# QCLovers/PyTDSCF

Measured on AMD Instinct MI355X. Metric: tdvp_sweeps_per_sec, higher is better.
Workload: dtype c128; 1 GPU; C4: synthetic exciton chain L=64 d=16 D=1024 M=32; L=64, d=16, D=1024, M=32, integrator=lanczos, steps_per_half_sweep=8, parallelism=single, approximate=False

## Files before the change

### include/mitdvp.h

```cpp
#ifndef MITDVP_H
#define MITDVP_H

#include <stddef.h>
#include <stdint.h>

#ifdef __cplusplus
extern "C" {
#endif

typedef struct mitdvp_engine mitdvp_engine;

enum {
  MITDVP_OK = 0,
  MITDVP_EINVAL = -1,
  MITDVP_EHIP = -2,
  MITDVP_ENOTCONV = -3,
  MITDVP_ESTATE = -4,
  MITDVP_ENOMEM = -5
};

enum { MITDVP_LANCZOS = 0, MITDVP_ARNOLDI = 1 };
enum { MITDVP_GAUGE_C = -1 , MITDVP_GAUGE_PSI = 0, MITDVP_GAUGE_A = 1, MITDVP_GAUGE_B = 2 };

typedef struct {
// ... 171 lines not shown
  double env_flops, env_ms;
  double keff_flops, keff_ms;
  double qr_flops, qr_ms;
  double krylov_vec_ms;
  long long n_heff, n_keff, n_env, n_qr;
  long long n_exp_site, n_exp_bond;
  long long n_launch;
  double heff_stage_ms[3];
  double n_collectives;
  double collective_bytes;
  double heff_flops_skipped;
  double n_host_waits;
  double n_heff_edge;
  double heff_stage_flops[3];
  double n_env_fold;
} mitdvp_counters;
int mitdvp_counters_get(mitdvp_engine* h, mitdvp_counters* out);
int mitdvp_counters_reset(mitdvp_engine* h);
int mitdvp_set_profiling(mitdvp_engine* h, int on);

int mitdvp_heff_apply(int device, const double* L, const double* W, const double* R, const double* psi,
                      int dl, int d, int dr, int ml, int mr, double* sigma_out, int reps, double* ms_out);
int mitdvp_keff_apply(int device, const double* L, const double* R, const double* sval,
                      int dl, int dr, int m, double* out);
int mitdvp_env_update(int device, int left, const double* env, const double* site, const double* W,
                      int dl, int d, int dr, int ml, int mr, double* out);
int mitdvp_gauge_trf(int device, int key, const double* psi, int dl, int d, int dr,
                     double* site_out, double* sigma_out);
int mitdvp_expm_dense(int device, int integrator, int conserve_norm, int lanczos_variant,
                      const double* mat, int n, const double* x, double scale_re, double scale_im,
// ... 39 lines not shown
```

### pytdscf_amd/_lib.py

```python

from __future__ import annotations

import ctypes as C
import os
import re

_HERE = os.path.dirname(os.path.abspath(__file__))
LIB_PATH = os.environ.get("MITDVP_LIB") or os.path.join(_HERE, "csrc", "libmitdvp.so")
HEADER_PATH = os.path.join(os.path.dirname(_HERE), "include", "mitdvp.h")

OK, EINVAL, EHIP, ENOTCONV, ESTATE, ENOMEM = 0, -1, -2, -3, -4, -5
LANCZOS, ARNOLDI = 0, 1
GAUGE_PSI, GAUGE_A, GAUGE_B, GAUGE_C = 0, 1, 2, -1


class MitdvpError(RuntimeError):
    pass


class Config(C.Structure):
    _fields_ = [
        ("nsite", C.c_int),
        ("device", C.c_int),
        ("integrator", C.c_int),
# ... 23 lines not shown
        ("n_heff", C.c_longlong),
        ("n_keff", C.c_longlong),
        ("n_env", C.c_longlong),
        ("n_qr", C.c_longlong),
        ("n_exp_site", C.c_longlong),
        ("n_exp_bond", C.c_longlong),
        ("n_launch", C.c_longlong),
        ("heff_stage_ms", C.c_double * 3),
        ("n_collectives", C.c_double),
        ("collective_bytes", C.c_double),
        ("heff_flops_skipped", C.c_double),
        ("n_host_waits", C.c_double),
        ("n_heff_edge", C.c_double),
        ("heff_stage_flops", C.c_double * 3),
        ("n_env_fold", C.c_double),
    ]

    def as_dict(self):
        d = {k: getattr(self, k) for k, _ in self._fields_ if k not in ("reserved", "heff_stage_ms", "heff_stage_flops")}
        d["heff_stage_ms"] = list(self.heff_stage_ms)
        d["heff_stage_flops"] = list(self.heff_stage_flops)
        return d


class BatchOut(C.Structure):

    _fields_ = [(k, C.POINTER(C.c_double)) for k in
                ("norm", "autocorr", "energy", "rdm", "mean_norm2", "mean_autocorr", "mean_energy", "mean_rdm")]


# ... 202 lines not shown
```

### pytdscf_amd/csrc/engine.h

```cpp
#pragma once
#include <functional>
#include <map>
#include <memory>
#include <string>
#include <vector>

#include "../../include/mitdvp.h"
#include "common.h"
#include "krylov_dev.h"
#include "qr.h"
#include "small_site.h"
#include "svd.h"
#include "vecops.h"

namespace mitdvp {

struct DevBuf {
  zc* p = nullptr;
  size_t n = 0;
  DevBuf() = default;
  DevBuf(const DevBuf&) = delete;
  DevBuf& operator=(const DevBuf&) = delete;
  DevBuf(DevBuf&& o) noexcept : p(o.p), n(o.n) { o.p = nullptr; o.n = 0; }
  DevBuf& operator=(DevBuf&& o) noexcept {
// ... 33 lines not shown
};

struct MpoSite {
  int ml = 0, d = 0, mr = 0;
  DevBuf w2l;
  DevBuf w2r;
  DevBuf w2lt, w2rt, kl_l, kl_r;
  int kl_stride_l = 0, kl_stride_r = 0;
  double sp_frac_l = 1.0, sp_frac_r = 1.0;
  struct SpSeg { int r0, r1; bool dense; int tile0; };
  std::vector<SpSeg> seg_l, seg_r;
  DevBuf w2el;
  DevBuf w2er;
  std::vector<hzc> whost;
  std::vector<char> nzblk;
  struct EnvFold { std::vector<int> t0; DevBuf ws, wg; };
  struct EdgeCache {
    bool valid = false;
    unsigned long long s = 0, e = 0;
    std::vector<hzc> lam, mu;
    bool has_l = false, has_r = false;
    int skip = 0;
    DevBuf w_l, w_r;
    DevBuf w_lf, w_rf;
    bool lf_ok = false, rf_ok = false;
    EnvFold envf[2];
    void rebuild(hipStream_t st, const MpoSite& w, unsigned long long S, unsigned long long E, const std::vector<hzc>& lam,
                 const std::vector<hzc>& mu);
  };
  mutable EdgeCache edge;
  DevBuf wtr;
// ... 71 lines not shown

  std::string last_error;

  void heff_apply(const zc* L, const MpoSite& w, const zc* R, const zc* psi, zc* out, int dl, int d, int dr,
                  hzc shift, const ApplyPlan& plan = {});
  void keff_apply(const zc* L, const zc* R, const zc* sig, zc* out, int d1, int d2, int m, hzc shift,
                  const KeffCompact* kc = nullptr);
  void heff_apply_rect(const zc* L, const MpoSite& w, const zc* R, const zc* psi, zc* out, int dlo, int dli, int d,
                       int dro, int dri, const ApplyPlan& plan = {});
  void heff_apply_edge(const zc* L, const MpoSite& w, const zc* R, const zc* psi, zc* out, int dl, int d, int dr,
                       const ApplyPlan& plan);
  ApplyPlan choose_apply_forms(const zc* Lb, const MpoSite& w, const zc* Rb, int dl, int d, int dr);
  void keff_apply_rect(const zc* L, const zc* R, const zc* sig, zc* out, int dlo, int dli, int dro, int dri, int m);
  void env_update_rect(const zc* env_in, const zc* Tk, const zc* Tb, const zc* w2, zc* env_out, int dbi, int dki,
                       int min_, int d, int dbo, int dko, int mout, const MpoSite* sp = nullptr, int sp_side = 0);
  bool env_fold_ok(const zc* env_in, int din, int min_, int d, int dout, int mout, const MpoSite* sp, int sp_side);
  void env_update_fold(const zc* env_in, const zc* T, zc* env_out, int din, int min_, int d, int dout, int mout,
                       const MpoSite::EnvFold& f);
  void env_update(const zc* env_in, const zc* T, const zc* w2, zc* env_out, int din, int min_, int d, int dout,
                  int mout, const zc* w2e = nullptr, const MpoSite* sp = nullptr, int sp_side = 0);
  template <class MV>
  int krylov_exp(hzc scale, MV&& matvec, zc* x, long n, int k_prev, long nsize = -1);
  template <class MV>
  int krylov_diag(MV&& matvec, zc* x, long n);
  void gauge_qr_left(const zc* psi, int dl, int d, int dr, zc* A_out, zc* sigma_out);
  void gauge_qr_right(const zc* psi, int dl, int d, int dr, zc* B_out, zc* Bt_out, zc* sigma_out);
  void ensure_work(long max_site, long max_x, long max_y, int max_qr_m, int max_qr_n, int qr_next = 0);
  void set_gate(int isite, const double* reim, int d);
  void apply_gates();
  void set_kraus(int isite, int two_site, const double* reim, int k, int d);
  void apply_kraus();
  double operate(int op_id, int maxstep, double conv_tol, int* iters_out);
  void set_adaptive(bool on, int dmax, int dd, double p_proj);
  void thin_to_full_A(const zc* A, int l, int c, int r, int e, zc* out);
  void thin_to_full_B(const zc* B, int l, int c, int r, int e, zc* out);
// ... 37 lines not shown
  const MpoSite& mpo(int op_id, int isite);
  mitdvp_config cfg;

 private:
  int ptr_mode_ = 0;
  struct CuClaim {
    int dev = -1, first = 0, count = 0;
    ~CuClaim() { if (dev >= 0) cu_range_release(dev, first, count); }
  } cu_claim_;
  bool qr_gauge_free_ = true;
  bool trim_identity_ = true;
  int edge_mode_ = -1;
  int fold_mode_ = -1;
  int strassen_mode_ = -1;
  bool strassen_batched_ = true;
  DevBuf str_l_, str_r_, str_v_, str_m_;
  static bool try_reserve(DevBuf& b, size_t elems);
  void strassen_side(const zc* fixed, bool fixed_is_a, const zc* psi, long ldpsi, zc* out, long hm, long hn, long hk, bool accumulate,
                     int level);
  int fold_env_mode_ = -1;
  struct EnvChecked { const MpoSite* w = nullptr; const zc* blk[2] = {nullptr, nullptr}; int n[2] = {0, 0}; } env_chk_;
  EnvChecked take_env_checked() { const EnvChecked c = env_chk_; env_chk_ = EnvChecked{}; return c; }
  struct IdentRecord { double dev[128]; hzc lam[128]; };
  static_assert(sizeof(IdentRecord) == 128 * 8 + 128 * 16 && sizeof(IdentRecord) <= 4 * NPART * sizeof(zc), "layout of the identity-check record");
  const IdentRecord& identity_sets(const zc* L, int ml, int dl, unsigned long long ms, const zc* R, int mr, int dr, unsigned long long me);
  void identity_blocks(const zc* L, int dl, int ml, const zc* R, int dr, int mr, bool* left, bool* right);
  int L_;
  hipStream_t st_ = nullptr;
  std::vector<int> dl_, dd_, dr_, gauge_;
  std::vector<DevBuf> site_;
  std::vector<std::vector<int>> sub_;
  std::vector<int> subn_;
  std::map<int, Operator> ops_;
  int center_ = -1;
  bool segment_ = false;
  int bnd_dl_ = 1, bnd_ml_ = 1, bnd_dr_ = 1, bnd_mr_ = 1;
// ... 115 lines not shown
```

### pytdscf_amd/csrc/engine.hip

```cpp
#include "engine_internal.h"
#include "engine_krylov.inc"
#include "rccl_dyn.h"

namespace mitdvp {

Engine::Engine(const mitdvp_config& c) : cfg(c), L_(c.nsite) {
  if (c.nsite < 1) throw ArgError("nsite must be >= 1");
  if (c.max_krylov < 1 || c.max_krylov > MAXK - 1) throw ArgError("max_krylov must be in [1, 20]");
  if (c.integrator != MITDVP_LANCZOS && c.integrator != MITDVP_ARNOLDI) throw ArgError("bad integrator");
  if (c.relax < 0 || c.relax > 2) throw ArgError("relax must be 0, 1 or 2");
  max_diag_krylov_ = c.max_diag_krylov > 0 ? c.max_diag_krylov : 64;
  if (const char* e = std::getenv("MITDVP_SMALL_KERNELS")) small_kernels_ = std::atoi(e) != 0;
  if (const char* e = std::getenv("MITDVP_SPARSE_W")) sparse_w_ = std::atoi(e) != 0;
  if (const char* e = std::getenv("MITDVP_TRIM_IDENTITY")) trim_identity_ = std::atoi(e) != 0;
  if (const char* e = std::getenv("MITDVP_EDGE_APPLY")) edge_mode_ = std::atoi(e);
  if (const char* e = std::getenv("MITDVP_FOLD_APPLY")) fold_mode_ = std::atoi(e);
  if (const char* e = std::getenv("MITDVP_FOLD_STRASSEN")) strassen_mode_ = std::atoi(e);
  if (const char* e = std::getenv("MITDVP_STRASSEN_BATCH")) strassen_batched_ = std::atoi(e) != 0;
  if (const char* e = std::getenv("MITDVP_FOLD_ENV")) fold_env_mode_ = std::atoi(e);
  if (const char* e = std::getenv("MITDVP_QR_GAUGE_FREE")) qr_gauge_free_ = std::atoi(e) != 0;
  if (const char* e = std::getenv("MITDVP_KEFF_IDENT")) keff_ident_ = std::atoi(e) != 0;
  int ndev = 0;
  HIP_CHECK(hipGetDeviceCount(&ndev));
  if (ndev < 1) throw HipError("no HIP device visible: the MI355X engine has no CPU fallback");
  if (c.device < 0 || c.device >= ndev) throw ArgError("bad device ordinal");
  HIP_CHECK(hipSetDevice(c.device));
  HIP_CHECK(hipDeviceGetAttribute(&n_cu_, hipDeviceAttributeMultiprocessorCount, c.device));
  if (c.cu_count > 0) {
    if (c.cu_first < 0 || c.cu_first + c.cu_count > n_cu_ || c.cu_count % 8 != 0 || c.cu_first % 8 != 0)
      throw ArgError("cu_first / cu_count: a multiple of 8 compute units inside the device (8 k units = k CUs on every XCD)");
    std::vector<uint32_t> mask((size_t)(n_cu_ + 31) / 32, 0u);
    for (int u = c.cu_first; u < c.cu_first + c.cu_count; ++u) mask[(size_t)u / 32] |= 1u << (u % 32);
    cu_range_claim(c.device, c.cu_first, c.cu_count);
    cu_claim_.dev = c.device; cu_claim_.first = c.cu_first; cu_claim_.count = c.cu_count;
// ... 279 lines not shown
  s.w2er.reserve(w2er.size());
  HIP_CHECK(hipMemcpyAsync(s.w2el.p, w2el.data(), w2el.size() * sizeof(zc), hipMemcpyHostToDevice, st_));
  HIP_CHECK(hipMemcpyAsync(s.w2er.p, w2er.data(), w2er.size() * sizeof(zc), hipMemcpyHostToDevice, st_));
  HIP_CHECK(hipStreamSynchronize(st_));
  s.set = true;
}

void Engine::set_mpo_core(int op_id, int isite, const double* reim, int ml, int dout, int din, int mr) {
  if (isite < 0 || isite >= L_) throw ArgError("set_mpo_core: bad site index");
  upload_mpo_core(op(op_id).sites[isite], reim, ml, dout, din, mr);
  if (op_id == 0) invalidate_env();
}
void Engine::set_shift(int op_id, double re, double im) { op(op_id).shift = hzc(re, im); }

void Engine::invalidate_env() {
  for (int b = 1; b < L_; ++b) {
    envL_ok_[b] = 0; envR_ok_[b] = 0;
    pool_put(std::move(envL_[b]));
    pool_put(std::move(envR_[b]));
  }
}

void Engine::ensure_work(long max_site, long max_x, long max_y, int max_qr_m, int max_qr_n, int qr_next) {
  X_.reserve(max_x);
  Y_.reserve(max_y);
  V_.reserve((size_t)MAXK * max_site);
  tmp1_.reserve(max_site);
  tmp2_.reserve(max_site);
  const size_t dd = (size_t)max_qr_n * max_qr_n;
  sig_.reserve(std::max<size_t>(dd, 1));
// ... 350 lines not shown
        cnt_.n_exp_bond += 1;
      }
      envR_ok_[p + 1] = 0;
      pool_put(std::move(envR_[p + 1]));
      ZgemmDesc g = zgemm_desc(sig_.p, site_[p + 1].p, spare.p, dr, dd_[p + 1] * dr_[p + 1], dr);
      zgemm(st_, g);
      cnt_.n_launch += 1;
      std::swap(site_[p + 1], spare);
      gauge_[p + 1] = MITDVP_GAUGE_PSI;
      center_ = p + 1;
    } else {
      gauge_qr_right(site_[p].p, dl, d, dr, spare.p, tmp2_.p, sig_.p);
      std::swap(site_[p], spare);
      gauge_[p] = MITDVP_GAUGE_B;
      envR_[p] = pool_get((size_t)dl * w.ml * dl);
      env_update(envR_[p + 1].p, tmp2_.p, w.w2r.p, envR_[p].p, dr, w.mr, d, dl, w.ml, w.w2er.p, &w, 1);
      envR_ok_[p] = 1;
      const zc* Lb = envL_[p].p;
      const zc* Rb = envR_[p].p;
      const int m = w.ml;
      if (cfg.relax != 2 && !small_bond_exp(p, Lb, Rb, dl, m, dt)) {
        const KeffCompact* kc = keff_prepare(Lb, Rb, dl, dl, m);
        auto mk = [&](const zc* in, zc* out) { keff_apply(Lb, Rb, in, out, dl, dl, m, shift, kc); };
        kprev_[p] = krylov_exp(scale_bond(dt), mk, sig_.p, (long)dl * dl, kprev_[p]);
        cnt_.n_exp_bond += 1;
      }
      envL_ok_[p] = 0;
      pool_put(std::move(envL_[p]));
      ZgemmDesc g = zgemm_desc(site_[p - 1].p, sig_.p, spare.p, dl_[p - 1] * dd_[p - 1], dl, dl);
      zgemm(st_, g);
      cnt_.n_launch += 1;
// ... 29 lines not shown
```

### pytdscf_amd/csrc/engine_apply.hip

```cpp
#include "engine_internal.h"

namespace mitdvp {

constexpr long STRASSEN_MIN_TILES = 256;

double Engine::w_stage(const MpoSite* sp, int side, const zc* w2, int d, int mout, int min_, int ncol, int nbatch) {
  ZgemmDesc g = zgemm_desc(w2, X_.p, Y_.p, d * mout, ncol, min_ * d);
  g.batch = nbatch; g.strideA = 0; g.strideB = (long)min_ * d * ncol; g.strideC = (long)d * mout * ncol;
  const bool use = sp && sparse_w_ && ncol >= 64 && (side == 0 ? sp->kl_l.p : sp->kl_r.p) &&
                   (side == 0 ? sp->sp_frac_l : sp->sp_frac_r) <= 0.6;
  if (!use) {
    zgemm(st_, g);
    return 1.0;
  }
  const zc* wt = side == 0 ? sp->w2lt.p : sp->w2rt.p;
  const int* kl = reinterpret_cast<const int*>(side == 0 ? sp->kl_l.p : sp->kl_r.p);
  const int stride = side == 0 ? sp->kl_stride_l : sp->kl_stride_r;
  const auto& segs = side == 0 ? sp->seg_l : sp->seg_r;
  const int K = min_ * d;
  for (int pass = 0; pass < 2; ++pass)
    for (const auto& sgm : segs) {
      if (sgm.dense != (pass == 0)) continue;
      ZgemmDesc h = g;
      h.A = wt + (size_t)sgm.r0 * K;
// ... 62 lines not shown
}

bool Engine::try_reserve(DevBuf& b, size_t elems) {
  if (elems <= b.n) return true;
  zc* q = nullptr;
  if (hipMalloc(&q, elems * sizeof(zc)) != hipSuccess) { (void)hipGetLastError(); return false; }
  b.release();
  b.p = q; b.n = elems;
  return true;
}

void Engine::strassen_side(const zc* fixed, bool fixed_is_a, const zc* psi, long ldpsi, zc* out, long hm, long hn, long hk,
                           bool accumulate, int level) {
  const long vr = fixed_is_a ? hk : hm, vc = fixed_is_a ? hn : hk;
  const int vset = fixed_is_a ? STRASSEN_B : STRASSEN_A;
  strassen_operands(st_, psi, ldpsi, vr, vc, str_v_.p, vset);
  int np = 7;
  long pm = hm, pn = hn, pk = hk;
  const zc* V = str_v_.p;
  zc* Mp = str_m_.p;
  if (level == 2) {
    zc* v2 = str_v_.p + 7 * vr * vc;
    strassen_operands(st_, str_v_.p, vc, vr / 2, vc / 2, v2, vset, 7, vr * vc, 7 * (vr / 2) * (vc / 2));
    np = 49; pm = hm / 2; pn = hn / 2; pk = hk / 2;
    V = v2;
    Mp = str_m_.p + 7 * hm * hn;
  }
  const zc* A = fixed_is_a ? fixed : V;
  const zc* B = fixed_is_a ? V : fixed;
  ZgemmDesc g = zgemm_desc(A, B, Mp, (int)pm, (int)pn, (int)pk);
  if (!fixed_is_a) { g.transB = 1; g.ldb = pk; }
  if (strassen_batched_) {
    g.batch = np; g.strideA = pm * pk; g.strideB = pk * pn; g.strideC = pm * pn;
    zgemm(st_, g);
  } else {
    for (int k = 0; k < np; ++k) {
      ZgemmDesc h = g;
      h.A = A + k * pm * pk; h.B = B + k * pk * pn; h.C = Mp + k * pm * pn;
      zgemm(st_, h);
    }
  }
  if (level == 2) strassen_combine(st_, Mp, pm, pn, str_m_.p, hn, false, 7, 7 * pm * pn, hm * hn);
  strassen_combine(st_, str_m_.p, hm, hn, out, ldpsi, accumulate);
  cnt_.n_launch += (level == 2 ? 4 : 2) + (strassen_batched_ ? 1 : np);
}

void Engine::heff_apply_edge(const zc* L, const MpoSite& w, const zc* R, const zc* psi, zc* out, int dl, int d, int dr,
                             const ApplyPlan& plan) {
  const int ml = w.ml, mr = w.mr;
  const MpoSite::EdgeCache& c = w.edge;
  bool first = true;
  double exe = 0.0;
  if (c.has_r && plan.fold_r && plan.strassen_r) {
    timer_begin(12);
    const bool two = plan.strassen_r == 2;
    strassen_side(str_r_.p, false, psi, (long)d * dr, out, dl / 2, (long)d * dr / 2, (long)d * dr / 2, false,
                  plan.strassen_r);
    timer_end();
    first = false;
// ... 134 lines not shown
        if (!w.nzblk[blk(in, out)]) continue;
        for (int i = 0; i < d; ++i)
          for (int j = 0; j < d; ++j) ws[((size_t)i * d + j) * mo + out] += wt[in] * Wel(in, i, j, out);
      }
    }
    for (size_t k = 0; k < f.t0.size(); ++k)
      for (int in = 0; in < mi; ++in) {
        if (((I >> in) & 1ull) || !w.nzblk[blk(in, f.t0[k])]) continue;
        for (int i = 0; i < d; ++i)
          for (int j = 0; j < d; ++j) wg[((k * d + i) * mi + in) * d + j] = Wel(in, i, j, f.t0[k]);
      }
    f.ws.reserve(ws.size());
    f.wg.reserve(wg.size());
    HIP_CHECK(hipMemcpyAsync(f.ws.p, ws.data(), ws.size() * sizeof(zc), hipMemcpyHostToDevice, st));
    HIP_CHECK(hipMemcpyAsync(f.wg.p, wg.data(), wg.size() * sizeof(zc), hipMemcpyHostToDevice, st));
    HIP_CHECK(hipStreamSynchronize(st));
  }
  HIP_CHECK(hipStreamSynchronize(st));
  s = S; e = E; this->lam = lam; this->mu = mu; valid = true;
}

ApplyPlan Engine::choose_apply_forms(const zc* Lb, const MpoSite& w, const zc* Rb, int dl, int d, int dr) {
  ApplyPlan plan;
  (void)take_env_checked();
  int a0, a1;
  const bool sharded = shard_range(dl, a0, a1);
  const int ml = w.ml, mr = w.mr;
  const bool can_fold_r = fold_mode_ != 0 && !sharded && (fold_mode_ > 0 || mr > d) && (size_t)d * dr * d * dr <= Y_.n;
  const bool can_fold_l = fold_mode_ != 0 && !sharded && (fold_mode_ > 0 || ml > d) && (size_t)dl * d * dl * d <= X_.n;
  const bool edge_cand = edge_mode_ != 0 && trim_identity_ && !w.whost.empty() && !sharded && dl >= 32 && dr >= 32 &&
// ... 35 lines not shown
  if (plan.fold_r || plan.fold_l) {
    timer_begin(11);
    if (plan.fold_r) fold_env_core(st_, Rb, w.edge.w_r.p, Y_.p, dr, mr, d, (long)d * mr, mr, 1, (long)dr * d * dr, (long)d * dr, dr, 1);
    if (plan.fold_l) fold_env_core(st_, Lb, w.edge.w_l.p, X_.p, dl, ml, d, (long)ml * d, 1, d, (long)dl * d, (long)d * dl * d, 1, d);
    const size_t quarter = (size_t)dl * d * dr / 4;
    auto tiles_fill = [](long pm, long pn) { return ((pm + 63) / 64) * ((pn + 63) / 64) >= STRASSEN_MIN_TILES; };
    auto level_of = [&](long rows, long cols, long klen) {
      if (strassen_mode_ == 0 || rows % 2 || cols % 2 || klen % 2) return 0;
      const bool four = rows % 4 == 0 && cols % 4 == 0 && klen % 4 == 0;
      if (strassen_mode_ > 0) return strassen_mode_ >= 2 && four ? 2 : 1;
      if (four && tiles_fill(rows / 4, cols / 4)) return 2;
      return tiles_fill(rows / 2, cols / 2) ? 1 : 0;
    };
    auto pack = [&](const zc* op, long n, DevBuf& f, int which, int want) {
      const long h = n / 2, q = n / 4;
      const size_t two = 7 * quarter + 49 * (quarter / 4);
      if (want == 2 && try_reserve(f, 49 * (size_t)q * q) && try_reserve(str_v_, two) && try_reserve(str_m_, two)) {
        strassen_operands2(st_, op, n, q, q, f.p, which);
        cnt_.n_launch += 1;
        return 2;
      }
      if (want == 0 || !try_reserve(f, 7 * (size_t)h * h) || !try_reserve(str_v_, 7 * quarter) || !try_reserve(str_m_, 7 * quarter))
        return 0;
      strassen_operands(st_, op, n, h, h, f.p, which);
      cnt_.n_launch += 1;
      return 1;
    };
    if (plan.fold_r) plan.strassen_r = pack(Y_.p, (long)d * dr, str_r_, STRASSEN_BT, level_of(dl, (long)d * dr, (long)d * dr));
    if (plan.fold_l) plan.strassen_l = pack(X_.p, (long)dl * d, str_l_, STRASSEN_A, level_of((long)dl * d, dr, (long)dl * d));
    timer_end();
    cnt_.n_launch += (plan.fold_r ? 1 : 0) + (plan.fold_l ? 1 : 0);
    if (std::getenv("MITDVP_EDGE_TRACE"))
      fprintf(stderr, "[mitdvp] folded sides of a site: R %s, L %s\n",
              plan.strassen_r == 2 ? "49 quarter-size products" : plan.strassen_r ? "seven half-size products" : plan.fold_r ? "plain product" : "not folded",
              plan.strassen_l == 2 ? "49 quarter-size products" : plan.strassen_l ? "seven half-size products" : plan.fold_l ? "plain product" : "not folded");
  }
  return plan;
}

void Engine::heff_apply(const zc* L, const MpoSite& w, const zc* R, const zc* psi, zc* out, int dl, int d, int dr,
                        hzc shift, const ApplyPlan& plan) {
  SmallChain sc;
  if (small_ok() && chain_heff(sc, L, w, R, dl, d, dr, false)) {
    timer_begin(10);
// ... 130 lines not shown
  }
  (void)w_stage(sp, sp_side, w2, d, mout, min_, dko, nm);
  {
    ZgemmDesc g = zgemm_desc(Tb + (size_t)m0 * d * dbo, Y_.p, env_out, dbo, mout * dko, nm * d);
    g.transA = 1; g.conjA = 1; g.lda = dbo;
    zgemm(st_, g);
  }
  timer_end();
  if (sharded) collective(COLL_ALLREDUCE, env_out, (size_t)dbo * mout * dko);
  cnt_.n_launch += 3;
  cnt_.n_env += 1;
  cnt_.env_flops += 8.0 * ((double)nm * dki * min_ * d * dko + (double)nm * dko * min_ * mout * d * d +
                           (double)nm * dbo * dko * mout * d);
}

bool Engine::env_fold_ok(const zc* env_in, int din, int min_, int d, int dout, int mout, const MpoSite* sp, int sp_side) {
  const EnvChecked chk = take_env_checked();
  int a0, a1;
  if (fold_env_mode_ == 0 || !sp || adaptive_ || shard_range(din, a0, a1)) return false;
  if (chk.w != sp || chk.blk[sp_side] != env_in || chk.n[sp_side] != din || !sp->edge.valid || sp->d != d) return false;
  if (min_ != (sp_side == 0 ? sp->ml : sp->mr) || mout != (sp_side == 0 ? sp->mr : sp->ml)) return false;
  if (min_ > 64 || mout > 64 || d > 64 || din > 65535 || dout > 65535) return false;
  const MpoSite::EnvFold& f = sp->edge.envf[sp_side];
  const double nt = (double)f.t0.size();
  if ((size_t)d * dout * d * dout > Y_.n || (size_t)din * d * dout > Y_.n || (nt > 0 && (size_t)din * d * din * d > X_.n)) return false;
  if (fold_env_mode_ > 0) return true;
  const double fresh = (double)d * d * dout * dout * din + nt * ((double)d * d * din * din * dout + (double)d * din * dout * dout);
  const double chain = (double)min_ * d * din * din * dout + (double)mout * d * din * dout * dout;
  return min_ > d && 4.0 * fresh <= 3.0 * chain;
}

void Engine::env_update_fold(const zc* env_in, const zc* T, zc* env_out, int din, int min_, int d, int dout, int mout,
                             const MpoSite::EnvFold& f) {
  timer_begin(1);
  const long ldg = (long)d * dout;
  for (int i = 0; i < d; ++i) {
    ZgemmDesc g = zgemm_desc(T + (size_t)i * dout, T + (size_t)i * dout, Y_.p + (size_t)i * dout * ldg + (size_t)i * dout, dout,
                             (d - i) * dout, din);
    g.transA = 1; g.conjA = 1; g.lda = ldg; g.ldb = ldg; g.ldc = ldg;
    zgemm(st_, g);
  }
  gram_mirror_lower(st_, Y_.p, dout, d);
  gram_env_core(st_, Y_.p, f.ws.p, env_out, dout, mout, d);
  for (size_t k = 0; k < f.t0.size(); ++k) {
    fold_env_core(st_, env_in, f.wg.p + k * (size_t)d * min_ * d, X_.p, din, min_, d, (long)min_ * d, 1, d, (long)din * d,
                  (long)d * din * d, 1, d);
    ZgemmDesc g = zgemm_desc(X_.p, T, Y_.p, din * d, dout, din * d);
    zgemm(st_, g);
    ZgemmDesc h = zgemm_desc(T, Y_.p, env_out + (size_t)f.t0[k] * dout, dout, dout, din * d);
    h.transA = 1; h.conjA = 1; h.lda = dout; h.ldc = (long)mout * dout; h.beta = make_double2(1.0, 0.0);
    zgemm(st_, h);
  }
  timer_end();
  cnt_.n_launch += d + (d > 1 ? 1 : 0) + 1 + 3 * (long long)f.t0.size();
  cnt_.n_env += 1;
  cnt_.n_env_fold += 1;
  cnt_.env_flops += 8.0 * ((double)din * din * min_ * d * dout + (double)din * dout * min_ * mout * d * d +
                           (double)din * dout * dout * mout * d);
}

void Engine::env_update(const zc* env_in, const zc* T, const zc* w2, zc* env_out, int din, int min_, int d, int dout,
                        int mout, const zc* w2e, const MpoSite* sp, int sp_side) {
  SmallChain sc;
  if (w2e && small_ok() && chain_env(sc, T, w2e, din, min_, d, dout, mout)) {
    timer_begin(1);
    small_apply(st_, ss_, sc, env_in, env_out, ss_partials(sc), make_double2(0.0, 0.0), false);
    timer_end();
    cnt_.n_launch += 1;
    cnt_.n_env += 1;
    cnt_.env_flops += 8.0 * ((double)din * din * min_ * d * dout + (double)din * dout * min_ * mout * d * d +
                             (double)din * dout * dout * mout * d);
    (void)take_env_checked();
    return;
  }
  if (env_fold_ok(env_in, din, min_, d, dout, mout, sp, sp_side)) {
    env_update_fold(env_in, T, env_out, din, min_, d, dout, mout, sp->edge.envf[sp_side]);
    return;
  }
  env_update_rect(env_in, T, T, w2, env_out, din, din, min_, d, dout, dout, mout, sp, sp_side);
}

void Engine::identity_blocks(const zc* L, int dl, int ml, const zc* R, int dr, int mr, bool* left, bool* right) {
  double* dev = reinterpret_cast<double*>(red_.p + RED_MISC);
  const double* h = reinterpret_cast<const double*>(h_red_.h + RED_MISC);
  if (L) ident_deviation(st_, L, (long)ml * dl, dl, dev);
  if (R) ident_deviation(st_, R + (size_t)(mr - 1) * dr, (long)mr * dr, dr, dev + 1);
  if (L || R) read_partials(RED_MISC, 1);
  *left = L && h[0] < 1e-13;
  *right = R && h[1] < 1e-13;
}

// ... 2 lines not shown
```

### pytdscf_amd/csrc/engine_segment.hip

```cpp
#include "engine_internal.h"
#include "engine_krylov.inc"

namespace mitdvp {

void Engine::replace_site(int i, const double* reim, int gauge) {
  if (i < 0 || i >= L_ || !site_[i].p) throw ArgError("replace_site: bad or unset site");
  const size_t e = (size_t)dl_[i] * dd_[i] * dr_[i];
  copy_in(site_[i].p, reim, e);
  gauge_[i] = gauge;
  if (gauge == MITDVP_GAUGE_PSI) center_ = i;
  else if (center_ == i) center_ = -1;
}

void Engine::reshape_site(int i, const double* reim, int l, int n, int r, int gauge) {
  if (i < 0 || i >= L_ || !site_[i].p) throw ArgError("reshape_site: bad or unset site");
  if (l < 1 || r < 1 || n != dd_[i]) throw ArgError("reshape_site: bad shape");
  if (i != 0 && i != L_ - 1) throw ArgError("reshape_site: only a block's first or last site faces a junction");
  if ((i > 0 && l != dl_[i]) || (i < L_ - 1 && r != dr_[i])) throw ArgError("reshape_site: only the outer bond may change");
  const size_t e = (size_t)l * n * r;
  site_[i].reserve(e);
  copy_in(site_[i].p, reim, e);
  dl_[i] = l; dr_[i] = r; gauge_[i] = gauge;
  if (gauge == MITDVP_GAUGE_PSI) center_ = i;
  else if (center_ == i) center_ = -1;
// ... 92 lines not shown
    cnt_.n_launch += nl; cnt_.n_qr += 1;
    std::swap(site_[p], spare);
    gauge_[p] = MITDVP_GAUGE_A;
    pool_put(std::move(envL_[p + 1]));
    envL_[p + 1] = pool_get((size_t)dr * w.mr * dr);
    env_update(envL_[p].p, site_[p].p, w.w2l.p, envL_[p + 1].p, dl, w.ml, d, dr, w.mr, w.w2el.p, &w, 0);
    envL_ok_[p + 1] = 1;
    bond_ = p + 1; bond_dim_ = dr;
  } else {
    if (!envR_ok_[p + 1]) throw ArgError("split_center: right environment missing");
    gauge_qr_right(site_[p].p, dl, d, dr, spare.p, tmp2_.p, sig_.p);
    std::swap(site_[p], spare);
    gauge_[p] = MITDVP_GAUGE_B;
    pool_put(std::move(envR_[p]));
    envR_[p] = pool_get((size_t)dl * w.ml * dl);
    env_update(envR_[p + 1].p, tmp2_.p, w.w2r.p, envR_[p].p, dr, w.mr, d, dl, w.ml, w.w2er.p, &w, 1);
    envR_ok_[p] = 1;
    bond_ = p; bond_dim_ = dl;
  }
  pool_put(std::move(spare));
  center_ = -1;
  bond_site_ = p;
}

void Engine::bond_exp(double dt) {
  require_ready();
  if (bond_ < 0) throw ArgError("bond_exp: no pending bond matrix (call split_center first)");
  const int b = bond_;
  if (!envL_ok_[b] || !envR_ok_[b]) throw ArgError("bond_exp: the environment blocks around the bond are not built");
  int d = 0, m = 0;
  env_shape(0, b, &d, &m);
// ... 155 lines not shown
```

### pytdscf_amd/csrc/vecops.h

```cpp
#pragma once
#include "common.h"

namespace mitdvp {

constexpr int NPART = 256;
constexpr int MAXK = 21;

constexpr int SMALL_VEC_EPT = 16;
constexpr long SMALL_VEC_N = 1024L * SMALL_VEC_EPT;

struct Coefs {
  zc c[MAXK];
};

int vec_blocks(long n);
void vec_dot(hipStream_t st, const zc* x, const zc* y, long n, bool conj_x, zc* out_p );
void vec_sumsq(hipStream_t st, const zc* x, long n, double* out_p );
void vec_lanczos_update(hipStream_t st, zc* v, const zc* vm1, const zc* vm2 , long n,
                        const zc* alpha_p, const double* betaprev_p, double* out_p);
void vec_lanczos_update_deferred(hipStream_t st, zc* v, const zc* ul, const zc* ulm1 , long n, const zc* alpha_raw_p,
                                 const double* nrm_all, int l, bool orthodox, double eps, double* out_p);
void vec_lanczos_step_small(hipStream_t st, zc* w, const zc* x, const zc* vl, const zc* vm2 , long n,
                            zc* alpha_p, const double* betaprev_p, double* nrm_p, double eps);
void vec_scale_inv_norm(hipStream_t st, zc* v, long n, const double* nrm_p, double eps);
// ... 7 lines not shown
void set_identity(hipStream_t st, zc* out, int rows, int cols, long ld);
void vec_copy_raw(hipStream_t st, zc* dst, const zc* src, size_t n);
void ident_deviation(hipStream_t st, const zc* blk, long ld, int n, double* out_dev);
void ident_deviation_multi(hipStream_t st, const zc* base, int nblk, long blk_stride, long ld, int n, double* out_dev,
                           zc* lam_dev, unsigned long long mask = ~0ull, bool clear = true);
void fold_env_core(hipStream_t st, const zc* env, const zc* w, zc* G, int n, int m, int d, long wi, long wj, long wm, long gi,
                   long gp, long gj, long gq);
void gram_env_core(hipStream_t st, const zc* G, const zc* ws, zc* out, int n, int m, int d);
void gram_mirror_lower(hipStream_t st, zc* G, int n, int d);
enum { STRASSEN_A = 0, STRASSEN_B = 1, STRASSEN_BT = 2 };
void strassen_operands(hipStream_t st, const zc* src, long ld, long hr, long hc, zc* dst, int which, int batch = 1,
                       long sstride = 0, long dstride = 0);
void strassen_operands2(hipStream_t st, const zc* src, long ld, long qr, long qc, zc* dst, int which);
void strassen_combine(hipStream_t st, const zc* M, long hr, long hc, zc* out, long ldo, bool accumulate, int batch = 1,
                      long mstride = 0, long ostride = 0);
void copy2d(hipStream_t st, zc* dst, long ldd, const zc* src, long lds, long rows, int cols, int zero_to, zc a,
            bool accumulate);
struct BlockList { int n; int idx[64]; zc f[64]; };
void gather_blocks(hipStream_t st, zc* dst, int n_dst, const zc* src, int m_src, long rows, int cols, const BlockList& bl);
void fill_scaled_blocks(hipStream_t st, zc* X, long ldx, int pos0, const zc* sig, long rows, int cols, const BlockList& bl);
void accum_scaled_blocks(hipStream_t st, zc* out, const zc* X, long ldx, const zc* sig, long rows, int cols, const BlockList& bl,
                         zc both);
void col_sumsq(hipStream_t st, const zc* x, long rows, int cols, double* out );
void row_sumsq(hipStream_t st, const zc* x, int rows, long cols, double* out );
void shell_sumsq(hipStream_t st, const zc* x, int n, double* out );
void transpose_batched(hipStream_t st, const zc* in, zc* out, int rows, int cols, long ldi, long ldo, int batch,
                       long in_bs, long out_bs);
void phys_diag(hipStream_t st, const zc* C, zc* out, int dl, int n, int dr, bool trace);
void permute_0213(hipStream_t st, const zc* in, zc* out, long n0, int n1, int n2, int n3);
void clock_probe(hipStream_t st, long iters, double* host_out3 );
// ... 7 lines not shown
```

### pytdscf_amd/csrc/vecops.hip

```cpp
#include "vecops.h"
#include "krylov_dev.h"

#include <algorithm>

namespace mitdvp {

__device__ __forceinline__ double wave_sum(double v) {
#pragma unroll
  for (int o = 32; o > 0; o >>= 1) v += __shfl_down(v, o, 64);
  return v;
}

__device__ __forceinline__ double block_sum(double v, double* sh ) {
  v = wave_sum(v);
  const int lane = threadIdx.x & 63, w = threadIdx.x >> 6;
  __syncthreads();
  if (lane == 0) sh[w] = v;
  __syncthreads();
  if (threadIdx.x == 0) sh[4] = sh[0] + sh[1] + sh[2] + sh[3];
  __syncthreads();
  return sh[4];
}

__device__ __forceinline__ zc sum_partials_z(const zc* p, int np, double* sh) {
// ... 1004 lines not shown
#pragma unroll
    for (int k = 0; k < 7; ++k) m[k] = M[k * blk + r * hc + c];
    zc o[4];
    o[0] = make_double2(((m[0].x + m[3].x) - m[4].x) + m[6].x, ((m[0].y + m[3].y) - m[4].y) + m[6].y);
    o[1] = make_double2(m[2].x + m[4].x, m[2].y + m[4].y);
    o[2] = make_double2(m[1].x + m[3].x, m[1].y + m[3].y);
    o[3] = make_double2(((m[0].x - m[1].x) + m[2].x) + m[5].x, ((m[0].y - m[1].y) + m[2].y) + m[5].y);
#pragma unroll
    for (int u = 0; u < 4; ++u) {
      zc* p = out + ((u >> 1) * hr + r) * ldo + (u & 1) * hc + c;
      if (acc) { const zc v = *p; o[u].x += v.x; o[u].y += v.y; }
      *p = o[u];
    }
  }
}
void strassen_operands(hipStream_t st, const zc* src, long ld, long hr, long hc, zc* dst, int which, int batch, long sstride,
                       long dstride) {
  if (hr < 1 || hc < 1 || batch < 1) return;
  if (ld < 2 * hc) throw ArgError("strassen_operands: leading dimension below the matrix width");
  if (which < 0 || which > 2) throw ArgError("strassen_operands: bad factor set");
  if (batch > 65535) throw ArgError("strassen_operands: batch above 65535");
  const dim3 grid((unsigned)((hc + 255) / 256), (unsigned)std::min<long>(hr, 32768), (unsigned)batch);
  if (which == STRASSEN_A)
    hipLaunchKernelGGL(k_strassen_operands<STRASSEN_A>, grid, dim3(256), 0, st, src, ld, hr, hc, dst, sstride, dstride);
  else if (which == STRASSEN_B)
    hipLaunchKernelGGL(k_strassen_operands<STRASSEN_B>, grid, dim3(256), 0, st, src, ld, hr, hc, dst, sstride, dstride);
  else hipLaunchKernelGGL(k_strassen_operands<STRASSEN_BT>, grid, dim3(256), 0, st, src, ld, hr, hc, dst, sstride, dstride);
  HIP_CHECK(hipGetLastError());
}
void strassen_operands2(hipStream_t st, const zc* src, long ld, long qr, long qc, zc* dst, int which) {
// ... 3 lines not shown
  const dim3 grid((unsigned)((qc + 255) / 256), (unsigned)std::min<long>(qr, 32768));
  if (which == STRASSEN_A) hipLaunchKernelGGL(k_strassen_operands2<STRASSEN_A>, grid, dim3(256), 0, st, src, ld, qr, qc, dst);
  else if (which == STRASSEN_B) hipLaunchKernelGGL(k_strassen_operands2<STRASSEN_B>, grid, dim3(256), 0, st, src, ld, qr, qc, dst);
  else hipLaunchKernelGGL(k_strassen_operands2<STRASSEN_BT>, grid, dim3(256), 0, st, src, ld, qr, qc, dst);
  HIP_CHECK(hipGetLastError());
}
void strassen_combine(hipStream_t st, const zc* M, long hr, long hc, zc* out, long ldo, bool accumulate, int batch, long mstride,
                      long ostride) {
  if (hr < 1 || hc < 1 || batch < 1) return;
  if (ldo < 2 * hc) throw ArgError("strassen_combine: leading dimension below the matrix width");
  if (batch > 65535) throw ArgError("strassen_combine: batch above 65535");
  const dim3 grid((unsigned)((hc + 255) / 256), (unsigned)std::min<long>(hr, 32768), (unsigned)batch);
  hipLaunchKernelGGL(k_strassen_combine, grid, dim3(256), 0, st, M, hr, hc, out, ldo, accumulate ? 1 : 0, mstride, ostride);
  HIP_CHECK(hipGetLastError());
}

void gram_env_core(hipStream_t st, const zc* G, const zc* ws, zc* out, int n, int m, int d) {
  if (n < 1 || d < 1) return;
  if (m < 1 || m > 64 || n > 65535 || d > 64) throw ArgError("gram_env_core: MPO bond in [1, 64], d <= 64 and bond dimension <= 65535");
  const dim3 grid((n + 63) / 64, n), block(256);
  const size_t lds = (size_t)d * 64 * sizeof(zc);
  if (m <= 16) hipLaunchKernelGGL(k_gram_env_core<4>, grid, block, lds, st, G, ws, out, n, m, d);
  else if (m <= 32) hipLaunchKernelGGL(k_gram_env_core<8>, grid, block, lds, st, G, ws, out, n, m, d);
  else hipLaunchKernelGGL(k_gram_env_core<16>, grid, block, lds, st, G, ws, out, n, m, d);
  HIP_CHECK(hipGetLastError());
}

}
```

Baseline: 0.04424 sweeps/s.

## Fuse two-level Strassen packing/combine and reuse Strassen operands in folded env update

Two-level Strassen now packs the variable operand in one step and combines the 49 products in a single kernel when the fixed operand is A. This removes an intermediate 7-block buffer and two launches. The folded environment update gains a reuse path: when the edge fold has a single term, it reuses the Strassen-packed operator from the Heff apply. That replaces the per-term fold_env_core plus zgemm chain with one Strassen product and one scaled zgemm, using a modified weight table. This adds state carried between the apply and the env update, plus new correctness conditions on the MPO sparsity pattern.

```diff
diff --git a/include/mitdvp.h b/include/mitdvp.h
--- a/include/mitdvp.h
+++ b/include/mitdvp.h
@@ -209,6 +209,7 @@
   double n_heff_edge;
   double heff_stage_flops[3];
   double n_env_fold;
+  double n_env_reuse;
 } mitdvp_counters;
 int mitdvp_counters_get(mitdvp_engine* h, mitdvp_counters* out);
 int mitdvp_counters_reset(mitdvp_engine* h);
diff --git a/pytdscf_amd/_lib.py b/pytdscf_amd/_lib.py
--- a/pytdscf_amd/_lib.py
+++ b/pytdscf_amd/_lib.py
@@ -61,6 +61,7 @@
         ("n_heff_edge", C.c_double),
         ("heff_stage_flops", C.c_double * 3),
         ("n_env_fold", C.c_double),
+        ("n_env_reuse", C.c_double),
     ]
 
     def as_dict(self):
diff --git a/pytdscf_amd/csrc/engine.h b/pytdscf_amd/csrc/engine.h
--- a/pytdscf_amd/csrc/engine.h
+++ b/pytdscf_amd/csrc/engine.h
@@ -71,7 +71,7 @@
   DevBuf w2er;
   std::vector<hzc> whost;
   std::vector<char> nzblk;
-  struct EnvFold { std::vector<int> t0; DevBuf ws, wg; };
+  struct EnvFold { std::vector<int> t0; DevBuf ws, wg; bool reuse = false; hzc reuse_alpha; DevBuf ws_reuse; };
   struct EdgeCache {
     bool valid = false;
     unsigned long long s = 0, e = 0;
@@ -173,11 +173,12 @@
   void keff_apply_rect(const zc* L, const zc* R, const zc* sig, zc* out, int dlo, int dli, int dro, int dri, int m);
   void env_update_rect(const zc* env_in, const zc* Tk, const zc* Tb, const zc* w2, zc* env_out, int dbi, int dki,
                        int min_, int d, int dbo, int dko, int mout, const MpoSite* sp = nullptr, int sp_side = 0);
-  bool env_fold_ok(const zc* env_in, int din, int min_, int d, int dout, int mout, const MpoSite* sp, int sp_side);
+  bool env_fold_ok(const zc* env_in, int din, int min_, int d, int dout, int mout, const MpoSite* sp, int sp_side,
+                   int* reuse_level);
   void env_update_fold(const zc* env_in, const zc* T, zc* env_out, int din, int min_, int d, int dout, int mout,
-                       const MpoSite::EnvFold& f);
+                       const MpoSite::EnvFold& f, int sp_side, int reuse_level, const zc* T_plain);
   void env_update(const zc* env_in, const zc* T, const zc* w2, zc* env_out, int din, int min_, int d, int dout,
-                  int mout, const zc* w2e = nullptr, const MpoSite* sp = nullptr, int sp_side = 0);
+                  int mout, const zc* w2e = nullptr, const MpoSite* sp = nullptr, int sp_side = 0, const zc* T_plain = nullptr);
   template <class MV>
   int krylov_exp(hzc scale, MV&& matvec, zc* x, long n, int k_prev, long nsize = -1);
   template <class MV>
@@ -245,12 +246,14 @@
   int fold_mode_ = -1;
   int strassen_mode_ = -1;
   bool strassen_batched_ = true;
+  bool strassen_fuse_ = true;
   DevBuf str_l_, str_r_, str_v_, str_m_;
   static bool try_reserve(DevBuf& b, size_t elems);
   void strassen_side(const zc* fixed, bool fixed_is_a, const zc* psi, long ldpsi, zc* out, long hm, long hn, long hk, bool accumulate,
                      int level);
   int fold_env_mode_ = -1;
-  struct EnvChecked { const MpoSite* w = nullptr; const zc* blk[2] = {nullptr, nullptr}; int n[2] = {0, 0}; } env_chk_;
+  bool env_reuse_ = true;
+  struct EnvChecked { const MpoSite* w = nullptr; const zc* blk[2] = {nullptr, nullptr}; int n[2] = {0, 0}; int lvl[2] = {0, 0}; } env_chk_;
   EnvChecked take_env_checked() { const EnvChecked c = env_chk_; env_chk_ = EnvChecked{}; return c; }
   struct IdentRecord { double dev[128]; hzc lam[128]; };
   static_assert(sizeof(IdentRecord) == 128 * 8 + 128 * 16 && sizeof(IdentRecord) <= 4 * NPART * sizeof(zc), "layout of the identity-check record");
diff --git a/pytdscf_amd/csrc/engine.hip b/pytdscf_amd/csrc/engine.hip
--- a/pytdscf_amd/csrc/engine.hip
+++ b/pytdscf_amd/csrc/engine.hip
@@ -17,7 +17,9 @@
   if (const char* e = std::getenv("MITDVP_FOLD_APPLY")) fold_mode_ = std::atoi(e);
   if (const char* e = std::getenv("MITDVP_FOLD_STRASSEN")) strassen_mode_ = std::atoi(e);
   if (const char* e = std::getenv("MITDVP_STRASSEN_BATCH")) strassen_batched_ = std::atoi(e) != 0;
+  if (const char* e = std::getenv("MITDVP_STRASSEN_FUSE")) strassen_fuse_ = std::atoi(e) != 0;
   if (const char* e = std::getenv("MITDVP_FOLD_ENV")) fold_env_mode_ = std::atoi(e);
+  if (const char* e = std::getenv("MITDVP_FOLD_ENV_REUSE")) env_reuse_ = std::atoi(e) != 0;
   if (const char* e = std::getenv("MITDVP_QR_GAUGE_FREE")) qr_gauge_free_ = std::atoi(e) != 0;
   if (const char* e = std::getenv("MITDVP_KEFF_IDENT")) keff_ident_ = std::atoi(e) != 0;
   int ndev = 0;
@@ -327,6 +329,7 @@
 void Engine::set_shift(int op_id, double re, double im) { op(op_id).shift = hzc(re, im); }
 
 void Engine::invalidate_env() {
+  (void)take_env_checked();
   for (int b = 1; b < L_; ++b) {
     envL_ok_[b] = 0; envR_ok_[b] = 0;
     pool_put(std::move(envL_[b]));
@@ -707,7 +710,7 @@
       std::swap(site_[p], spare);
       gauge_[p] = MITDVP_GAUGE_B;
       envR_[p] = pool_get((size_t)dl * w.ml * dl);
-      env_update(envR_[p + 1].p, tmp2_.p, w.w2r.p, envR_[p].p, dr, w.mr, d, dl, w.ml, w.w2er.p, &w, 1);
+      env_update(envR_[p + 1].p, tmp2_.p, w.w2r.p, envR_[p].p, dr, w.mr, d, dl, w.ml, w.w2er.p, &w, 1, site_[p].p);
       envR_ok_[p] = 1;
       const zc* Lb = envL_[p].p;
       const zc* Rb = envR_[p].p;
diff --git a/pytdscf_amd/csrc/engine_apply.hip b/pytdscf_amd/csrc/engine_apply.hip
--- a/pytdscf_amd/csrc/engine_apply.hip
+++ b/pytdscf_amd/csrc/engine_apply.hip
@@ -100,17 +100,23 @@
                            bool accumulate, int level) {
   const long vr = fixed_is_a ? hk : hm, vc = fixed_is_a ? hn : hk;
   const int vset = fixed_is_a ? STRASSEN_B : STRASSEN_A;
-  strassen_operands(st_, psi, ldpsi, vr, vc, str_v_.p, vset);
+  const bool fused = level == 2 && strassen_fuse_ && fixed_is_a;
   int np = 7;
   long pm = hm, pn = hn, pk = hk;
   const zc* V = str_v_.p;
   zc* Mp = str_m_.p;
-  if (level == 2) {
-    zc* v2 = str_v_.p + 7 * vr * vc;
-    strassen_operands(st_, str_v_.p, vc, vr / 2, vc / 2, v2, vset, 7, vr * vc, 7 * (vr / 2) * (vc / 2));
+  if (fused) {
+    strassen_operands2(st_, psi, ldpsi, vr / 2, vc / 2, str_v_.p, vset);
     np = 49; pm = hm / 2; pn = hn / 2; pk = hk / 2;
-    V = v2;
-    Mp = str_m_.p + 7 * hm * hn;
+  } else {
+    strassen_operands(st_, psi, ldpsi, vr, vc, str_v_.p, vset);
+    if (level == 2) {
+      zc* v2 = str_v_.p + 7 * vr * vc;
+      strassen_operands(st_, str_v_.p, vc, vr / 2, vc / 2, v2, vset, 7, vr * vc, 7 * (vr / 2) * (vc / 2));
+      np = 49; pm = hm / 2; pn = hn / 2; pk = hk / 2;
+      V = v2;
+      Mp = str_m_.p + 7 * hm * hn;
+    }
   }
   const zc* A = fixed_is_a ? fixed : V;
   const zc* B = fixed_is_a ? V : fixed;
@@ -126,9 +132,13 @@
       zgemm(st_, h);
     }
   }
-  if (level == 2) strassen_combine(st_, Mp, pm, pn, str_m_.p, hn, false, 7, 7 * pm * pn, hm * hn);
-  strassen_combine(st_, str_m_.p, hm, hn, out, ldpsi, accumulate);
-  cnt_.n_launch += (level == 2 ? 4 : 2) + (strassen_batched_ ? 1 : np);
+  if (fused) {
+    strassen_combine2(st_, Mp, pm, pn, out, ldpsi, accumulate);
+  } else {
+    if (level == 2) strassen_combine(st_, Mp, pm, pn, str_m_.p, hn, false, 7, 7 * pm * pn, hm * hn);
+    strassen_combine(st_, str_m_.p, hm, hn, out, ldpsi, accumulate);
+  }
+  cnt_.n_launch += (fused ? 2 : level == 2 ? 4 : 2) + (strassen_batched_ ? 1 : np);
 }
 
 void Engine::heff_apply_edge(const zc* L, const MpoSite& w, const zc* R, const zc* psi, zc* out, int dl, int d, int dr,
@@ -293,6 +303,26 @@
     f.wg.reserve(wg.size());
     HIP_CHECK(hipMemcpyAsync(f.ws.p, ws.data(), ws.size() * sizeof(zc), hipMemcpyHostToDevice, st));
     HIP_CHECK(hipMemcpyAsync(f.wg.p, wg.data(), wg.size() * sizeof(zc), hipMemcpyHostToDevice, st));
+    f.reuse = false;
+    std::vector<hzc> ws2;
+    if (f.t0.size() == 1) {
+      const int o = f.t0[0];
+      const hzc wo = side == 0 ? mu[o] : lam[o];
+      bool ok = (((side == 0 ? E : S) >> o) & 1ull) && wo != hzc(0.0, 0.0);
+      if (side == 1)
+        for (int c = 0; c < ml && ok; ++c) {
+          if (c == o || !((S >> c) & 1ull) || lam[c] == hzc(0.0, 0.0)) continue;
+          for (int t = 0; t < mr && ok; ++t) if (w.nzblk[(size_t)c * mr + t]) ok = false;
+        }
+      if (ok) {
+        f.reuse = true;
+        f.reuse_alpha = hzc(1.0, 0.0) / wo;
+        ws2 = ws;
+        if (side == 1) for (int ij = 0; ij < d * d; ++ij) ws2[(size_t)ij * mo + o] = hzc(0.0, 0.0);
+        f.ws_reuse.reserve(ws2.size());
+        HIP_CHECK(hipMemcpyAsync(f.ws_reuse.p, ws2.data(), ws2.size() * sizeof(zc), hipMemcpyHostToDevice, st));
+      }
+    }
     HIP_CHECK(hipStreamSynchronize(st));
   }
   HIP_CHECK(hipStreamSynchronize(st));
@@ -358,7 +388,7 @@
     };
     auto pack = [&](const zc* op, long n, DevBuf& f, int which, int want) {
       const long h = n / 2, q = n / 4;
-      const size_t two = 7 * quarter + 49 * (quarter / 4);
+      const size_t two = (strassen_fuse_ && which == STRASSEN_A ? 0 : 7 * quarter) + 49 * (quarter / 4);
       if (want == 2 && try_reserve(f, 49 * (size_t)q * q) && try_reserve(str_v_, two) && try_reserve(str_m_, two)) {
         strassen_operands2(st_, op, n, q, q, f.p, which);
         cnt_.n_launch += 1;
@@ -372,6 +402,8 @@
     };
     if (plan.fold_r) plan.strassen_r = pack(Y_.p, (long)d * dr, str_r_, STRASSEN_BT, level_of(dl, (long)d * dr, (long)d * dr));
     if (plan.fold_l) plan.strassen_l = pack(X_.p, (long)dl * d, str_l_, STRASSEN_A, level_of((long)dl * d, dr, (long)dl * d));
+    env_chk_.lvl[0] = plan.strassen_l;
+    env_chk_.lvl[1] = plan.strassen_r;
     timer_end();
     cnt_.n_launch += (plan.fold_r ? 1 : 0) + (plan.fold_l ? 1 : 0);
     if (std::getenv("MITDVP_EDGE_TRACE"))
@@ -532,8 +564,10 @@
                            (double)nm * dbo * dko * mout * d);
 }
 
-bool Engine::env_fold_ok(const zc* env_in, int din, int min_, int d, int dout, int mout, const MpoSite* sp, int sp_side) {
+bool Engine::env_fold_ok(const zc* env_in, int din, int min_, int d, int dout, int mout, const MpoSite* sp, int sp_side,
+                         int* reuse_level) {
   const EnvChecked chk = take_env_checked();
+  *reuse_level = 0;
   int a0, a1;
   if (fold_env_mode_ == 0 || !sp || adaptive_ || shard_range(din, a0, a1)) return false;
   if (chk.w != sp || chk.blk[sp_side] != env_in || chk.n[sp_side] != din || !sp->edge.valid || sp->d != d) return false;
@@ -542,6 +576,7 @@
   const MpoSite::EnvFold& f = sp->edge.envf[sp_side];
   const double nt = (double)f.t0.size();
   if ((size_t)d * dout * d * dout > Y_.n || (size_t)din * d * dout > Y_.n || (nt > 0 && (size_t)din * d * din * d > X_.n)) return false;
+  if (env_reuse_ && f.reuse) *reuse_level = chk.lvl[sp_side];
   if (fold_env_mode_ > 0) return true;
   const double fresh = (double)d * d * dout * dout * din + nt * ((double)d * d * din * din * dout + (double)d * din * dout * dout);
   const double chain = (double)min_ * d * din * din * dout + (double)mout * d * din * dout * dout;
@@ -549,7 +584,8 @@
 }
 
 void Engine::env_update_fold(const zc* env_in, const zc* T, zc* env_out, int din, int min_, int d, int dout, int mout,
-                             const MpoSite::EnvFold& f) {
+                             const MpoSite::EnvFold& f, int sp_side, int reuse_level, const zc* T_plain) {
+  const bool reuse = reuse_level >= 1;
   timer_begin(1);
   const long ldg = (long)d * dout;
   for (int i = 0; i < d; ++i) {
@@ -559,8 +595,20 @@
     zgemm(st_, g);
   }
   gram_mirror_lower(st_, Y_.p, dout, d);
-  gram_env_core(st_, Y_.p, f.ws.p, env_out, dout, mout, d);
-  for (size_t k = 0; k < f.t0.size(); ++k) {
+  gram_env_core(st_, Y_.p, reuse ? f.ws_reuse.p : f.ws.p, env_out, dout, mout, d);
+  const zc alpha = make_double2(f.reuse_alpha.real(), f.reuse_alpha.imag());
+  if (reuse && sp_side == 0) {
+    strassen_side(str_l_.p, true, T, dout, Y_.p, (long)din * d / 2, dout / 2, (long)din * d / 2, false, reuse_level);
+    ZgemmDesc h = zgemm_desc(T, Y_.p, env_out + (size_t)f.t0[0] * dout, dout, dout, din * d);
+    h.transA = 1; h.conjA = 1; h.lda = dout; h.ldc = (long)mout * dout; h.alpha = alpha; h.beta = make_double2(1.0, 0.0);
+    zgemm(st_, h);
+  } else if (reuse) {
+    strassen_side(str_r_.p, false, T_plain, (long)d * din, Y_.p, dout / 2, (long)d * din / 2, (long)d * din / 2, false, reuse_level);
+    ZgemmDesc h = zgemm_desc(T_plain, Y_.p, env_out + (size_t)f.t0[0] * dout, dout, dout, d * din);
+    h.conjA = 1; h.transB = 1; h.ldb = (long)d * din; h.ldc = (long)mout * dout; h.alpha = alpha; h.beta = make_double2(1.0, 0.0);
+    zgemm(st_, h);
+  }
+  for (size_t k = 0; !reuse && k < f.t0.size(); ++k) {
     fold_env_core(st_, env_in, f.wg.p + k * (size_t)d * min_ * d, X_.p, din, min_, d, (long)min_ * d, 1, d, (long)din * d,
                   (long)d * din * d, 1, d);
     ZgemmDesc g = zgemm_desc(X_.p, T, Y_.p, din * d, dout, din * d);
@@ -570,15 +618,16 @@
     zgemm(st_, h);
   }
   timer_end();
-  cnt_.n_launch += d + (d > 1 ? 1 : 0) + 1 + 3 * (long long)f.t0.size();
+  cnt_.n_launch += d + (d > 1 ? 1 : 0) + 1 + (reuse ? 1 : 3 * (long long)f.t0.size());
   cnt_.n_env += 1;
   cnt_.n_env_fold += 1;
+  if (reuse) cnt_.n_env_reuse += 1;
   cnt_.env_flops += 8.0 * ((double)din * din * min_ * d * dout + (double)din * dout * min_ * mout * d * d +
                            (double)din * dout * dout * mout * d);
 }
 
 void Engine::env_update(const zc* env_in, const zc* T, const zc* w2, zc* env_out, int din, int min_, int d, int dout,
-                        int mout, const zc* w2e, const MpoSite* sp, int sp_side) {
+                        int mout, const zc* w2e, const MpoSite* sp, int sp_side, const zc* T_plain) {
   SmallChain sc;
   if (w2e && small_ok() && chain_env(sc, T, w2e, din, min_, d, dout, mout)) {
     timer_begin(1);
@@ -591,8 +640,10 @@
     (void)take_env_checked();
     return;
   }
-  if (env_fold_ok(env_in, din, min_, d, dout, mout, sp, sp_side)) {
-    env_update_fold(env_in, T, env_out, din, min_, d, dout, mout, sp->edge.envf[sp_side]);
+  int reuse_level = 0;
+  if (env_fold_ok(env_in, din, min_, d, dout, mout, sp, sp_side, &reuse_level)) {
+    if (sp_side == 1 && !T_plain) reuse_level = 0;
+    env_update_fold(env_in, T, env_out, din, min_, d, dout, mout, sp->edge.envf[sp_side], sp_side, reuse_level, T_plain);
     return;
   }
   env_update_rect(env_in, T, T, w2, env_out, din, din, min_, d, dout, dout, mout, sp, sp_side);
diff --git a/pytdscf_amd/csrc/engine_segment.hip b/pytdscf_amd/csrc/engine_segment.hip
--- a/pytdscf_amd/csrc/engine_segment.hip
+++ b/pytdscf_amd/csrc/engine_segment.hip
@@ -130,7 +130,7 @@
     gauge_[p] = MITDVP_GAUGE_B;
     pool_put(std::move(envR_[p]));
     envR_[p] = pool_get((size_t)dl * w.ml * dl);
-    env_update(envR_[p + 1].p, tmp2_.p, w.w2r.p, envR_[p].p, dr, w.mr, d, dl, w.ml, w.w2er.p, &w, 1);
+    env_update(envR_[p + 1].p, tmp2_.p, w.w2r.p, envR_[p].p, dr, w.mr, d, dl, w.ml, w.w2er.p, &w, 1, site_[p].p);
     envR_ok_[p] = 1;
     bond_ = p; bond_dim_ = dl;
   }
diff --git a/pytdscf_amd/csrc/vecops.h b/pytdscf_amd/csrc/vecops.h
--- a/pytdscf_amd/csrc/vecops.h
+++ b/pytdscf_amd/csrc/vecops.h
@@ -45,6 +45,7 @@
 void strassen_operands2(hipStream_t st, const zc* src, long ld, long qr, long qc, zc* dst, int which);
 void strassen_combine(hipStream_t st, const zc* M, long hr, long hc, zc* out, long ldo, bool accumulate, int batch = 1,
                       long mstride = 0, long ostride = 0);
+void strassen_combine2(hipStream_t st, const zc* M, long qr, long qc, zc* out, long ldo, bool accumulate);
 void copy2d(hipStream_t st, zc* dst, long ldd, const zc* src, long lds, long rows, int cols, int zero_to, zc a,
             bool accumulate);
 struct BlockList { int n; int idx[64]; zc f[64]; };
diff --git a/pytdscf_amd/csrc/vecops.hip b/pytdscf_amd/csrc/vecops.hip
--- a/pytdscf_amd/csrc/vecops.hip
+++ b/pytdscf_amd/csrc/vecops.hip
@@ -1042,6 +1042,41 @@
     }
   }
 }
+__global__ __launch_bounds__(256) void k_strassen_combine2(const zc* __restrict__ M, long qr, long qc, zc* __restrict__ out,
+                                                           long ldo, int acc) {
+  const long c = (long)blockIdx.x * 256 + threadIdx.x;
+  if (c >= qc) return;
+  const long blk = qr * qc;
+  for (long r = blockIdx.y; r < qr; r += gridDim.y) {
+    zc h[7][4];
+#pragma unroll
+    for (int k1 = 0; k1 < 7; ++k1) {
+      zc m[7];
+      const zc* mk = M + 7 * k1 * blk + r * qc + c;
+      asm volatile("" : "+v"(mk));
+#pragma unroll
+      for (int k = 0; k < 7; ++k) m[k] = mk[k * blk];
+      h[k1][0] = make_double2(((m[0].x + m[3].x) - m[4].x) + m[6].x, ((m[0].y + m[3].y) - m[4].y) + m[6].y);
+      h[k1][1] = make_double2(m[2].x + m[4].x, m[2].y + m[4].y);
+      h[k1][2] = make_double2(m[1].x + m[3].x, m[1].y + m[3].y);
+      h[k1][3] = make_double2(((m[0].x - m[1].x) + m[2].x) + m[5].x, ((m[0].y - m[1].y) + m[2].y) + m[5].y);
+    }
+#pragma unroll
+    for (int u = 0; u < 4; ++u) {
+      zc o[4];
+      o[0] = make_double2(((h[0][u].x + h[3][u].x) - h[4][u].x) + h[6][u].x, ((h[0][u].y + h[3][u].y) - h[4][u].y) + h[6][u].y);
+      o[1] = make_double2(h[2][u].x + h[4][u].x, h[2][u].y + h[4][u].y);
+      o[2] = make_double2(h[1][u].x + h[3][u].x, h[1][u].y + h[3][u].y);
+      o[3] = make_double2(((h[0][u].x - h[1][u].x) + h[2][u].x) + h[5][u].x, ((h[0][u].y - h[1][u].y) + h[2][u].y) + h[5][u].y);
+#pragma unroll
+      for (int U = 0; U < 4; ++U) {
+        zc* p = out + ((2 * (U >> 1) + (u >> 1)) * qr + r) * ldo + (2 * (U & 1) + (u & 1)) * qc + c;
+        if (acc) { const zc v = *p; o[U].x += v.x; o[U].y += v.y; }
+        *p = o[U];
+      }
+    }
+  }
+}
 void strassen_operands(hipStream_t st, const zc* src, long ld, long hr, long hc, zc* dst, int which, int batch, long sstride,
                        long dstride) {
   if (hr < 1 || hc < 1 || batch < 1) return;
@@ -1075,6 +1110,13 @@
   hipLaunchKernelGGL(k_strassen_combine, grid, dim3(256), 0, st, M, hr, hc, out, ldo, accumulate ? 1 : 0, mstride, ostride);
   HIP_CHECK(hipGetLastError());
 }
+void strassen_combine2(hipStream_t st, const zc* M, long qr, long qc, zc* out, long ldo, bool accumulate) {
+  if (qr < 1 || qc < 1) return;
+  if (ldo < 4 * qc) throw ArgError("strassen_combine2: leading dimension below the matrix width");
+  const dim3 grid((unsigned)((qc + 255) / 256), (unsigned)std::min<long>(qr, 32768));
+  hipLaunchKernelGGL(k_strassen_combine2, grid, dim3(256), 0, st, M, qr, qc, out, ldo, accumulate ? 1 : 0);
+  HIP_CHECK(hipGetLastError());
+}
 
 void gram_env_core(hipStream_t st, const zc* G, const zc* ws, zc* out, int n, int m, int d) {
   if (n < 1 || d < 1) return;
```

Result: faster. 0.04551 sweeps/s, median of 6 (+2.9%).
